# visionworkbench/visionworkbench

Hardware: AMD Instinct MI355X
Metric: disparity Mpix/s, 4096x4096 pair, 7x7 SAD, +-64-px search (higher is better)
Workload: dtype u8

## Files before the change

### visionworkbench_amd/csrc/bm_sad_u8.hip

```cpp
#include <climits>
#include <cstdlib>
#include <type_traits>

#include "vwgpu_internal.h"
#include "u8_tile.h"

#ifdef VWGPU_TILE_STAMPS
__device__ unsigned long long* g_sad_stamps = nullptr;
extern "C" int vwgpu_debug_set_sad_stamps(void* d_buf) {
  unsigned long long* p = static_cast<unsigned long long*>(d_buf);
  return hipMemcpyToSymbol(HIP_SYMBOL(g_sad_stamps), &p, sizeof p) == hipSuccess ? 0 : -3;
}
#define VWGPU_STAMP(k) do { if (g_sad_stamps && tid == 0) g_sad_stamps[(size_t)wg * 16 + (k)] = wall_clock64(); } while (0)
#else
#define VWGPU_STAMP(k) do { } while (0)
#endif

namespace {

using namespace vwgpu_u8;
typedef uint32_t u32;
typedef uint64_t u64;
typedef unsigned short u16x2 __attribute__((ext_vector_type(2)));

__device__ __forceinline__ u32 pk_sub_u16(u32 a, u32 b) {
  return __builtin_bit_cast(u32, (u16x2)(__builtin_bit_cast(u16x2, a) - __builtin_bit_cast(u16x2, b)));
}
__device__ __forceinline__ u32 pk_max_u16(u32 a, u32 b) {
  return __builtin_bit_cast(u32, __builtin_elementwise_max(__builtin_bit_cast(u16x2, a), __builtin_bit_cast(u16x2, b)));
}
__device__ __forceinline__ u32 pk_min_u16(u32 a, u32 b) {
  return __builtin_bit_cast(u32, __builtin_elementwise_min(__builtin_bit_cast(u16x2, a), __builtin_bit_cast(u16x2, b)));
}
__device__ __forceinline__ void umin3_acc(u32& k, u32 a, u32 b) {
  asm volatile("v_min3_u32 %0, %0, %1, %2" : "+v"(k) : "v"(a), "v"(b));
}

template <int W>
__device__ __forceinline__ void key_sub(u32& key, u32 a, u32 b) {
  if (W == 0)
    asm volatile("v_sub_u16_sdwa %0, %1, %2 dst_sel:WORD_1 dst_unused:UNUSED_PRESERVE src0_sel:WORD_0 src1_sel:WORD_0"
                 : "+v"(key) : "v"(a), "v"(b));
  else
    asm volatile("v_sub_u16_sdwa %0, %1, %2 dst_sel:WORD_1 dst_unused:UNUSED_PRESERVE src0_sel:WORD_1 src1_sel:WORD_1"
                 : "+v"(key) : "v"(a), "v"(b));
}

template <int KX, int KY, int TY, int WV = 0>
struct Cfg {
  static constexpr int NW = (KX + 3) / 4;
  static constexpr int EW = NW <= 2 ? 2 : 4;
  static constexpr int WAVES = WV ? WV : (NW <= 2 ? 4 : 2);
  static constexpr int THREADS = WAVES * 64;
  static constexpr int TWB = WAVES * 256;
  static constexpr int NR = TY + KY - 1;
  static constexpr int LBW = TWB / 4 + NW + 1;
  static constexpr u32 LAST_MASK = (KX % 4 == 0) ? 0xffffffffu : ((1u << (8 * (KX % 4))) - 1u);
};

__device__ __forceinline__ void divmod_small(int idx, int d, float inv, int& quo, int& rem) {
  int qq = (int)(((float)idx + 0.5f) * inv);
  int rr = idx - qq * d;
  if (rr < 0) { --qq; rr += d; }
  if (rr >= d) { ++qq; rr -= d; }
  quo = qq; rem = rr;
}

__device__ __forceinline__ bool sad_second_on_cu(unsigned block, int first_round) {
  return (int)(block >> 3) >= (first_round >> 4);
}

__host__ __device__ constexpr size_t ent_words(int nr, int ne, int ew, int gr, int ty, int pt) {
  const size_t ent = (size_t)nr * ne * ew;
  const size_t merge = gr > 1 ? (size_t)(gr - 1) * (ty / gr) * 4 * pt + (size_t)gr * pt : 0;
  const size_t ob = (size_t)gr * (pt / 64) * 768;
  return ent > merge ? (ent > ob ? ent : ob) : (merge > ob ? merge : ob);
}

template <int KX, int KY, int TY, int GR, int WV = 0, bool EM = true>
__global__ void __launch_bounds__((GR * (Cfg<KX, KY, TY, WV>::THREADS)), (GR > 1 ? 1 : (TY <= 8 && KX <= 8 ? 3 : 2)))
bm_sad_u8_kernel(const float* __restrict__ L, ptrdiff_t ls, int lw, int lh,
                 const float* __restrict__ R, ptrdiff_t rs, int rcw, int rch,
                 int sx, int sy, int ne, int32_t* __restrict__ out, ptrdiff_t os, int ow, int oh,
                 int* __restrict__ flag_set, int* __restrict__ flag_clear,
                 int gxt, int ntiles, int last_round, int first_round, int stagger_ticks) {
  typedef Cfg<KX, KY, TY, WV> C;
  constexpr bool SPLIT = GR > 1;
  constexpr int NW = C::NW, EW = C::EW, NR = C::NR;
  constexpr int NRP = EM ? (NR | 1) : NR;
  extern __shared__ __attribute__((aligned(16))) u32 lds[];
  u32* ent = lds;
  const int bpitch = ne + NW + 1;
  u32* base = lds + ent_words(NRP, ne, EW, GR, TY, C::THREADS);
  u32* item_ctr = base + (size_t)NR * bpitch;

  constexpr int PT = C::THREADS;
  constexpr int NT = GR * PT;
  const int tid = threadIdx.x;
  const int grp = SPLIT ? __builtin_amdgcn_readfirstlane(tid / PT) : 0;
  const int ltid = SPLIT ? tid % PT : tid;
  const int pair_id = __builtin_amdgcn_readfirstlane(ltid >> 6);
  const int per_xcd = gridDim.x >> 3;
  const int wg = (int)(blockIdx.x & 7) * per_xcd + (int)(blockIdx.x >> 3);
  if (wg >= ntiles) return;
  const int x0 = (wg % gxt) * C::TWB;
  const int y0 = (wg / gxt) * TY;
  const int q = x0 + 4 * ltid;
  u32 bad_acc = 0;
  if (wg == 0 && tid == 0) *flag_clear = 0;
#ifdef VWGPU_TILE_STAMPS
  if (g_sad_stamps && tid == 0) {
    unsigned hw, xcc;
    asm volatile("s_getreg_b32 %0, hwreg(HW_REG_HW_ID)" : "=s"(hw));
    asm volatile("s_getreg_b32 %0, hwreg(HW_REG_XCC_ID)" : "=s"(xcc));
    unsigned long long* rec = g_sad_stamps + (size_t)wg * 16;
    rec[0] = wall_clock64(); rec[1] = clock64(); rec[2] = ((unsigned long long)xcc << 32) | hw;
  }
#endif

  if (!SPLIT && (int)blockIdx.x < first_round && sad_second_on_cu(blockIdx.x, first_round)) {
    if (tid < 64) {
      const u64 t_start = wall_clock64();
      for (int it = 0; it < 512 && wall_clock64() - t_start < (u64)stagger_ticks; ++it) __builtin_amdgcn_s_sleep(8);
    }
    __syncthreads();
  }
  stage_u8_rows<NR>(L, ls, lw, lh, x0, y0, C::LBW, C::LBW, ent, tid, NT, bad_acc);
  stage_u8_rows<NR>(R, rs, rcw, rch, x0, y0, bpitch, bpitch, base, tid, NT, bad_acc);
  __syncthreads();
  u64 win[NR][NW];
#pragma unroll
  for (int r = 0; r < NR; ++r) {
    u32 a[NW + 1];
#pragma unroll
    for (int n = 0; n <= NW; ++n) a[n] = ent[r * C::LBW + ltid + n];
#pragma unroll
    for (int n = 0; n < NW; ++n) win[r][n] = (u64)a[n] | ((u64)a[n + 1] << 32);
  }

  VWGPU_STAMP(3);
  u32 K[TY][4];
  u32 MN[TY][2], MX[TY][2];
#pragma unroll
  for (int y = 0; y < TY; ++y) K[y][0] = K[y][1] = K[y][2] = K[y][3] = 0xffffffffu;
  u32 eq_rows = (1u << TY) - 1u;
  int eq_checks = 0;
  constexpr int NPROBE = 4;
  const u32 zero = 0;

  const bool late = !SPLIT && (int)blockIdx.x >= last_round;
  if (!SPLIT) { if (late) __builtin_amdgcn_s_setprio(2); else __builtin_amdgcn_s_setprio(3); }
  typedef std::true_type T;
  typedef std::false_type F;

  auto sweep = [&](auto max_tag) __attribute__((always_inline)) {
    constexpr bool MAXSWEEP = decltype(max_tag)::value;
    for (int dy = 0; dy < sy; ++dy) {
      __syncthreads();
      if (dy > 0 || (MAXSWEEP && sy > 1)) stage_u8_rows<NR>(R, rs, rcw, rch, x0, y0 + dy, bpitch, bpitch, base, tid, NT, bad_acc);
      for (int t = 0; t < 4; ++t) {
        const int a_last = (sx + 2 - t) >> 2;
        __syncthreads();
        if (!MAXSWEEP && !SPLIT && dy == 0 && late) {
          if (t == 2) __builtin_amdgcn_s_setprio(1);
          else if (t == 3) __builtin_amdgcn_s_setprio(0);
        }
        {
          auto build = [&](int r, int m) __attribute__((always_inline)) {
            const u32* bp = base + (size_t)r * bpitch + m;
            u32 b[NW + 1];
#pragma unroll
            for (int n = 0; n <= NW; ++n) b[n] = bp[n];
            u32 w[EW];
#pragma unroll
            for (int n = 0; n < EW; ++n) w[n] = 0;
#pragma unroll
            for (int n = 0; n < NW; ++n) w[n] = __builtin_amdgcn_alignbyte(b[n + 1], b[n], t);
            w[NW - 1] &= C::LAST_MASK;
            u32* e = ent + (EM ? (size_t)m * NRP + r : (size_t)r * ne + m) * EW;
            if (EW == 2) *reinterpret_cast<uint2*>(e) = make_uint2(w[0], w[1]);
            else *reinterpret_cast<uint4*>(e) = make_uint4(w[0], w[1], w[2 % EW], w[3 % EW]);
          };
#pragma unroll 4
          for (int r = grp; r < NR; r += NT / PT) build(r, ltid);
          const int rem = ne - PT, total = NR * rem;
          const float inv = 1.0f / (float)rem;
          for (int idx = tid; idx < total; idx += NT) {
            int r, m;
            divmod_small(idx, rem, inv, r, m);
            build(r, PT + m);
          }
          if (SPLIT && tid < PT / 64) item_ctr[tid] = 0u;
        }
        __syncthreads();

        auto step = [&](int a, auto masked_tag, auto pair_tag, auto probe_tag) __attribute__((always_inline)) {
          constexpr bool MASKED = decltype(masked_tag)::value;
          constexpr bool PAIR = decltype(pair_tag)::value;
          constexpr bool PROBE = decltype(probe_tag)::value;
          const int jbase = 4 * a + t;
          const int ibase = dy * sx + jbase;
          u32 kinA[4], kinB[4];
          u32 orA[2] = {0u, 0u};
#pragma unroll
          for (int i = 0; i < 4; ++i) {
            kinA[i] = (u32)(ibase - i) & 0xffffu;
            kinB[i] = (u32)(ibase + 4 - i) & 0xffffu;
            if (MASKED) {
              const int d = jbase - i;
              if (d < 0 || d >= sx) orA[i >> 1] |= (i & 1) ? 0xffff0000u : 0x0000ffffu;
            }
          }
          const u32* ep = ent + (size_t)(ltid + a) * (EM ? NRP * EW : EW);
          u64 accA = 0, accB = 0;
          u64 PA[NR], PB[NR];
          constexpr int PF = 4;
          u32 wa[NR][EW], wb[NR][EW];
          auto fetch = [&](int r) __attribute__((always_inline)) {
            const u32* e = ep + (EM ? (size_t)r * EW : (size_t)r * ne * EW);
            constexpr int NX = EM ? NRP * EW : EW;
            if (EW == 2) {
              const uint2 v = *reinterpret_cast<const uint2*>(e);
              wa[r][0] = v.x; wa[r][1] = v.y;
              if (PAIR) { const uint2 u = *reinterpret_cast<const uint2*>(e + NX); wb[r][0] = u.x; wb[r][1] = u.y; }
            } else {
              const uint4 v = *reinterpret_cast<const uint4*>(e);
              wa[r][0] = v.x; wa[r][1] = v.y; wa[r][2 % EW] = v.z; wa[r][3 % EW] = v.w;
              if (PAIR) { const uint4 u = *reinterpret_cast<const uint4*>(e + NX); wb[r][0] = u.x; wb[r][1] = u.y; wb[r][2 % EW] = u.z; wb[r][3 % EW] = u.w; }
            }
          };
#pragma unroll
          for (int r = 0; r < PF && r < NR; ++r) fetch(r);
#pragma unroll
          for (int r = 0; r < NR; ++r) {
            if (r + PF < NR) fetch(r + PF);
#pragma unroll
            for (int n = 0; n < NW; ++n) {
              accA = __builtin_amdgcn_qsad_pk_u16_u8(win[r][n], wa[r][n], accA);
              if (PAIR) accB = __builtin_amdgcn_qsad_pk_u16_u8(win[r][n], wb[r][n], accB);
            }
            PA[r] = accA;
            if (PAIR) PB[r] = accB;
            if (r >= KY - 1) {
              const int y = r - (KY - 1);
              const int ro = (r >= KY) ? r - KY : 0;
              const u32 nA0 = (u32)PA[r], nA1 = (u32)(PA[r] >> 32);
              const u32 oA0 = (r >= KY) ? (u32)PA[ro] : zero;
              const u32 oA1 = (r >= KY) ? (u32)(PA[ro] >> 32) : zero;
              if (MAXSWEEP) {
                const u32 sA0 = pk_sub_u16(nA0, oA0), sA1 = pk_sub_u16(nA1, oA1);
                MN[y][0] = pk_min_u16(MN[y][0], MASKED ? (sA0 | orA[0]) : sA0);
                MN[y][1] = pk_min_u16(MN[y][1], MASKED ? (sA1 | orA[1]) : sA1);
                MX[y][0] = pk_max_u16(MX[y][0], MASKED ? (sA0 & ~orA[0]) : sA0);
                MX[y][1] = pk_max_u16(MX[y][1], MASKED ? (sA1 & ~orA[1]) : sA1);
                if (PAIR) {
                  const u32 nB0 = (u32)PB[r], nB1 = (u32)(PB[r] >> 32);
                  const u32 oB0 = (r >= KY) ? (u32)PB[ro] : zero;
                  const u32 oB1 = (r >= KY) ? (u32)(PB[ro] >> 32) : zero;
                  const u32 sB0 = pk_sub_u16(nB0, oB0), sB1 = pk_sub_u16(nB1, oB1);
                  MN[y][0] = pk_min_u16(MN[y][0], sB0);
                  MN[y][1] = pk_min_u16(MN[y][1], sB1);
                  MX[y][0] = pk_max_u16(MX[y][0], sB0);
                  MX[y][1] = pk_max_u16(MX[y][1], sB1);
                }
              } else {
                key_sub<0>(kinA[0], nA0, oA0); key_sub<1>(kinA[1], nA0, oA0);
                key_sub<0>(kinA[2], nA1, oA1); key_sub<1>(kinA[3], nA1, oA1);
                if (PAIR) {
                  const u32 nB0 = (u32)PB[r], nB1 = (u32)(PB[r] >> 32);
                  const u32 oB0 = (r >= KY) ? (u32)PB[ro] : zero;
                  const u32 oB1 = (r >= KY) ? (u32)(PB[ro] >> 32) : zero;
                  key_sub<0>(kinB[0], nB0, oB0); key_sub<1>(kinB[1], nB0, oB0);
                  key_sub<0>(kinB[2], nB1, oB1); key_sub<1>(kinB[3], nB1, oB1);
                  if (PROBE) {
                    u32 x[4];
#pragma unroll
                    for (int i = 0; i < 4; ++i) {
                      asm volatile("v_xor_b32 %0, %1, %2" : "=v"(x[i]) : "v"(kinA[i]), "v"(kinB[i]));
                      x[i] = (q + i < ow) ? x[i] : 0xffffffffu;
                    }
                    const u32 m01 = x[0] < x[1] ? x[0] : x[1], m23 = x[2] < x[3] ? x[2] : x[3];
                    if ((m01 < m23 ? m01 : m23) >> 16) eq_rows &= ~(1u << y);
                  }
                  umin3_acc(K[y][0], kinA[0], kinB[0]);
                  umin3_acc(K[y][1], kinA[1], kinB[1]);
                  umin3_acc(K[y][2], kinA[2], kinB[2]);
                  umin3_acc(K[y][3], kinA[3], kinB[3]);
                } else {
                  const u32 kA0 = (MASKED && (orA[0] & 0x0000ffffu)) ? 0xffffffffu : kinA[0];
                  const u32 kA1 = (MASKED && (orA[0] & 0xffff0000u)) ? 0xffffffffu : kinA[1];
                  const u32 kA2 = (MASKED && (orA[1] & 0x0000ffffu)) ? 0xffffffffu : kinA[2];
                  const u32 kA3 = (MASKED && (orA[1] & 0xffff0000u)) ? 0xffffffffu : kinA[3];
                  umin3_acc(K[y][0], kA0, kA0);
                  umin3_acc(K[y][1], kA1, kA1);
                  umin3_acc(K[y][2], kA2, kA2);
                  umin3_acc(K[y][3], kA3, kA3);
                }
              }
            }
          }
        };

        int a_lo = (t >= 3) ? 0 : 1;
        int a_hi = (sx - 1 - t >= 0) ? ((sx - 1 - t) >> 2) + 1 : 0;
        if (a_hi > a_last + 1) a_hi = a_last + 1;
        if (a_lo > a_hi) a_lo = a_hi;
        const int n1 = a_lo;
        const int npair = (a_hi - n1) > 0 ? (a_hi - n1) >> 1 : 0;
        int nprobe = 0;
        if (!MAXSWEEP && dy == 0 && t == 0) nprobe = npair < NPROBE - eq_checks ? npair : NPROBE - eq_checks;
        const int a4 = n1 + 2 * npair;
        const int n4 = a_last - a4 + 1 > 0 ? a_last - a4 + 1 : 0;
        const int nitems = n1 + npair + n4;
        int seq = 0;
        auto next_item = [&]() __attribute__((always_inline)) -> int {
          if (MAXSWEEP) return grp == 0 ? seq++ : 0x7fffffff;
          if (!SPLIT) return seq++;
          int lane, v = 0;
          asm volatile("v_mbcnt_lo_u32_b32 %0, -1, 0\n\tv_mbcnt_hi_u32_b32 %0, -1, %0" : "=v"(lane));
          if (lane == 0) v = (int)atomicAdd(&item_ctr[pair_id], 1u);
          return __builtin_amdgcn_readfirstlane(v);
        };
        int i = next_item();
        for (; i < n1; i = next_item()) step(i, T{}, F{}, F{});
        for (; i < n1 + nprobe; i = next_item()) step(n1 + 2 * (i - n1), F{}, T{}, T{});
        for (; i < n1 + npair; i = next_item()) step(n1 + 2 * (i - n1), F{}, T{}, F{});
        for (; i < nitems; i = next_item()) step(a4 + (i - n1 - npair), T{}, F{}, F{});
        eq_checks += nprobe;
        if (!MAXSWEEP && dy == 0) VWGPU_STAMP(4 + t);
      }
    }
  };
  sweep(F{});
  if (!SPLIT) __builtin_amdgcn_s_setprio(3);

  if (bad_acc != 0u) atomicOr(flag_set, 1);
  constexpr int RG = TY / GR;
  static_assert(TY % GR == 0, "rows per group");
  auto row_mine = [&](int y) __attribute__((always_inline)) -> bool { return !SPLIT || (y / RG == grp); };
  if (SPLIT) {
    u32* xk = ent;
    u32* xe = ent + (size_t)(GR - 1) * RG * 4 * PT;
    u32 eq_all = eq_rows;
#pragma unroll
    for (int d = 0; d < GR; ++d) {
      __syncthreads();
      if (grp != d) {
        const int slot = grp < d ? grp : grp - 1;
#pragma unroll
        for (int y = 0; y < RG; ++y)
#pragma unroll
          for (int s2 = 0; s2 < 4; ++s2) xk[((slot * RG + y) * 4 + s2) * PT + ltid] = K[d * RG + y][s2];
      }
      if (d == 0) xe[grp * PT + ltid] = eq_rows;
      __syncthreads();
      if (grp == d) {
#pragma unroll
        for (int slot = 0; slot < GR - 1; ++slot)
#pragma unroll
          for (int y = 0; y < RG; ++y)
#pragma unroll
            for (int s2 = 0; s2 < 4; ++s2) {
              const u32 o = xk[((slot * RG + y) * 4 + s2) * PT + ltid];
              K[d * RG + y][s2] = o < K[d * RG + y][s2] ? o : K[d * RG + y][s2];
            }
      }
      if (d == 0) {
#pragma unroll
        for (int g2 = 0; g2 < GR; ++g2) eq_all &= xe[g2 * PT + ltid];
      }
    }
    eq_rows = eq_all;
  }
  u32 cand = eq_checks < NPROBE ? (1u << TY) - 1u : eq_rows;
#pragma unroll
  for (int y = 0; y < TY; ++y)
    if (y0 + y >= oh || q >= ow || !row_mine(y)) cand &= ~(1u << y);
  const int any = __syncthreads_or(cand != 0u);

  {
    const int wv = ltid >> 6, lane = ltid & 63;
    u32* ob = ent + (size_t)(grp * (PT / 64) + wv) * 768;
    const int xw = x0 + 256 * wv;
    int nd = (ow - xw) * 3;
    nd = nd < 0 ? 0 : (nd > 768 ? 768 : nd);
    const u32 sx_magic = sx > 1 ? (u32)(0xffffffffu / (u32)sx) + 1u : 0u;
    struct __attribute__((packed, aligned(4))) U4 { u32 x, y, z, w; };
#pragma unroll
    for (int y = 0; y < TY; ++y) {
      const int oy = y0 + y;
      if (oy >= oh || !row_mine(y)) continue;
      u32 v[12];
#pragma unroll
      for (int s = 0; s < 4; ++s) {
        const u32 di = K[y][s] & 0xffffu;
        u32 dx, dy;
        if (sy == 1) { dx = di; dy = 0; }
        else { dy = sx == 1 ? di : __umulhi(di, sx_magic); dx = di - dy * (u32)sx; }
        v[3 * s] = dx;
        v[3 * s + 1] = dy;
        v[3 * s + 2] = 0x7fffffffu;
      }
      uint4* ow4 = reinterpret_cast<uint4*>(ob + lane * 12);
      ow4[0] = make_uint4(v[0], v[1], v[2], v[3]);
      ow4[1] = make_uint4(v[4], v[5], v[6], v[7]);
      ow4[2] = make_uint4(v[8], v[9], v[10], v[11]);
      int32_t* orow = out + ((ptrdiff_t)oy * os + xw) * 3;
#pragma unroll
      for (int k = 0; k < 3; ++k) {
        const int idx = k * 256 + lane * 4;
        const uint4 t = *reinterpret_cast<const uint4*>(ob + idx);
        if (idx + 3 < nd) {
          U4 u; u.x = t.x; u.y = t.y; u.z = t.z; u.w = t.w;
          *reinterpret_cast<U4*>(orow + idx) = u;
        } else {
          if (idx < nd) orow[idx] = (int32_t)t.x;
          if (idx + 1 < nd) orow[idx + 1] = (int32_t)t.y;
          if (idx + 2 < nd) orow[idx + 2] = (int32_t)t.z;
        }
      }
    }
  }

#ifdef VWGPU_TILE_STAMPS
  if (g_sad_stamps && tid == 0) { g_sad_stamps[(size_t)wg * 16 + 8] = wall_clock64(); g_sad_stamps[(size_t)wg * 16 + 9] = clock64(); }
#endif
  if (__builtin_expect(!any, 1)) return;
#pragma unroll
  for (int y = 0; y < TY; ++y) {
    MN[y][0] = MN[y][1] = 0xffffffffu;
    MX[y][0] = MX[y][1] = 0u;
  }
  sweep(T{});
  if (grp == 0) {
#pragma unroll
    for (int y = 0; y < TY; ++y) {
      const u32 same0 = MN[y][0] ^ MX[y][0], same1 = MN[y][1] ^ MX[y][1];
      const bool inv[4] = {(same0 & 0xffffu) == 0, (same0 >> 16) == 0, (same1 & 0xffffu) == 0, (same1 >> 16) == 0};
#pragma unroll
      for (int s = 0; s < 4; ++s)
        if (inv[s] && y0 + y < oh && q + s < ow)
          out[((ptrdiff_t)(y0 + y) * os + q + s) * 3 + 2] = 0;
    }
  }
}

typedef void (*KernelFn)(const float*, ptrdiff_t, int, int, const float*, ptrdiff_t, int, int, int, int, int,
                         int32_t*, ptrdiff_t, int, int, int*, int*, int, int, int, int, int);
struct Launch {
  int kx, ky, ty;
  int threads, twb, nr, ew, nw;
  int split_groups;
  KernelFn fn;
  KernelFn split_fn;
  KernelFn fn_rm, split_fn_rm;
};

template <bool ON, int KX, int KY, int TY, int GR, int WV, bool EM>
constexpr KernelFn kernel_if() {
  if constexpr (ON) return bm_sad_u8_kernel<KX, KY, TY, GR, WV, EM>;
  else return nullptr;
}

template <int KX, int KY, int TY, bool WITH_SPLIT = false, int WV = 0>
constexpr Launch make_launch() {
  typedef Cfg<KX, KY, TY, WV> C;
  return Launch{KX, KY, TY, C::THREADS, C::TWB, C::NR, C::EW, C::NW, WV ? 4 : 2,
                kernel_if<WV == 0, KX, KY, TY, 1, WV, true>(),
                kernel_if<WITH_SPLIT, KX, KY, TY, (WV ? 4 : 2), WV, true>(),
                kernel_if<WV == 0, KX, KY, TY, 1, WV, false>(),
                kernel_if<WITH_SPLIT, KX, KY, TY, (WV ? 4 : 2), WV, false>()};
}

const Launch kLaunch[] = {
    make_launch<3, 3, 16>(), make_launch<5, 5, 16>(), make_launch<7, 7, 16, true>(), make_launch<7, 7, 8, true>(), make_launch<7, 7, 16, true, 2>(),
    make_launch<7, 5, 16>(), make_launch<9, 9, 12>(), make_launch<11, 11, 8>(),
};

const Launch* find_launch(int kx, int ky) {
  for (const Launch& l : kLaunch)
    if (l.kx == kx && l.ky == ky) return &l;
  return nullptr;
}

const Launch* pick_launch(int kx, int ky, int ow, int oh, int num_cu, int groups, bool* split) {
  const Launch* best = nullptr;
  double best_cost = 0.0;
  *split = false;
  if (groups == 3) {
    bool has = false;
    for (const Launch& l : kLaunch) has |= l.kx == kx && l.ky == ky && l.split_fn && !l.fn;
    if (!has) groups = 0;
  }
  for (const Launch& l : kLaunch) {
    if (l.kx != kx || l.ky != ky) continue;
    const long long wgs = (long long)((ow + l.twb - 1) / l.twb) * ((oh + l.ty - 1) / l.ty);
    const double n = (double)((wgs + num_cu - 1) / num_cu);
    const int resident = (l.ty <= 8 && l.kx <= 8) ? 3 : 2;
    const bool narrow = l.twb * 2 <= 4 * 256 && l.split_fn && !l.fn;
    const double wfrac = narrow ? 0.5 : 1.0;
    for (int sp = 0; sp < 2; ++sp) {
      if (sp && !l.split_fn) continue;
      if (!sp && !l.fn) continue;
      if (groups == 3 && !narrow) continue;
      if (groups && groups != 3 && (narrow || (l.split_fn && (groups == 2) != (sp == 1)))) continue;
      const double steps = (sp ? l.nr * 0.55 * n : (n < 2.0 ? l.nr * 0.74 : l.nr * 0.5 * n)) * wfrac;
      const double rounds = sp ? n : (double)(((long long)n + resident - 1) / resident);
      const double cost = steps + (narrow ? 5.7 : 4.5) * rounds;
      if (!best || cost < best_cost) { best = &l; best_cost = cost; *split = sp != 0; }
    }
  }
  return best;
}

constexpr size_t kMaxLds = 80 * 1024;

constexpr int kStaggerTicks = 1400;

int entries_per_row(const Launch& l, int sx) { return l.twb / 4 + ((sx + 2) >> 2) + 1; }

size_t lds_bytes(const Launch& l, int sx, int groups, bool em) {
  const int ne = entries_per_row(l, sx);
  const size_t ent = ent_words(em ? (l.nr | 1) : l.nr, ne, l.ew, groups, l.ty, l.threads);
  const size_t left = (size_t)l.nr * (l.twb / 4 + l.nw + 1);
  const size_t base = (size_t)l.nr * (ne + l.nw + 1);
  return ((ent > left ? ent : left) + base) * sizeof(u32);
}

bool supported(const vwgpu_bm_args& a) {
  if (a.cost_type != VWGPU_ABSOLUTE_DIFFERENCE) return false;
  const Launch* l = find_launch(a.kx, a.ky);
  if (!l) return false;
  if ((long long)a.sx * a.sy > 65535) return false;
  return lds_bytes(*l, a.sx, l->split_fn ? l->split_groups : 1, false) <= kMaxLds;
}

int launch(vwgpu_ctx* ctx, const vwgpu_bm_args& a, int** d_flag) {
  const int kx = a.kx, sx = a.sx, sy = a.sy, ow = a.ow(), oh = a.oh();
  bool split = false;
  const int plan_cu = ctx->sad_round_slots > 0 ? (ctx->sad_round_slots + 1) / 2 : ctx->num_cu;
  const Launch* l = pick_launch(kx, a.ky, ow, oh, plan_cu, ctx->sad_groups, &split);
  if (!l) return vwgpu_fail(ctx, VWGPU_ERR_NOIMPL, "no packed-u8 kernel for %dx%d", kx, a.ky);
  const int rcw = a.lw + sx - 1, rch = a.lh + sy - 1;
  const int gx = (ow + l->twb - 1) / l->twb, gy = (oh + l->ty - 1) / l->ty;
  const int ne = entries_per_row(*l, sx);
  const int groups = split ? l->split_groups : 1;
  const size_t ctr_bytes = split ? 64 : 0;
  const bool em = ctx->sad_layout == 0 && lds_bytes(*l, sx, groups, true) + ctr_bytes <= kMaxLds;
  const size_t shmem = lds_bytes(*l, sx, groups, em) + ctr_bytes;
  ctx->sad_last_launch = l->ty | (l->twb / 256) << 8 | groups << 12 | (em ? 1 : 0) << 16;
  const KernelFn main_fn = em ? (split ? l->split_fn : l->fn) : (split ? l->split_fn_rm : l->fn_rm);
  const unsigned grid1 = (unsigned)((gx * gy + 7) / 8 * 8);
  const int resident = (l->ty <= 8 && l->kx <= 8) ? 3 : 2;
  const int slots = ctx->sad_round_slots > 0 ? ctx->sad_round_slots : ctx->num_cu * resident;
  const bool rounds = !split && (int)grid1 >= 2 * slots;
  const int last_round = rounds ? (int)grid1 - slots : INT_MAX;
  const int first_round = (rounds && resident == 2) ? slots : 0;
  vwgpu_flag_pair f;
  int rc = vwgpu_packed_prologue(ctx, reinterpret_cast<const void*>(main_fn), shmem, d_flag, &f);
  if (rc) return rc;
  {
    vwgpu_prof_scope ps(ctx, "bm_sad_u8");
    hipLaunchKernelGGL(main_fn, dim3(grid1), dim3(split ? l->split_groups * l->threads : l->threads), shmem, ctx->stream,
                       a.left, a.ls, a.lw, a.lh, a.right, a.rs, rcw, rch, sx, sy, ne, a.out, a.os, ow, oh,
                       f.set, f.clear, gx, gx * gy, last_round, first_round, kStaggerTicks);
  }
  VWGPU_HIP(ctx, hipGetLastError());
  return VWGPU_OK;
}

}

vwgpu_bm_matcher vwgpu_bm_sad_u8 = {VWGPU_PATH_SAD_U8, 7, "packed-u8", supported, launch};
```

### visionworkbench_amd/csrc/u8_tile.h

```cpp
#pragma once
#include <hip/hip_runtime.h>
#include <cstdint>

namespace vwgpu_u8 {

typedef uint32_t u32;

__device__ __forceinline__ u32 pack4_check(float4 v, u32& acc) {
  u32 p = 0;
  p = __builtin_amdgcn_cvt_pk_u8_f32(v.x, 0, p);
  p = __builtin_amdgcn_cvt_pk_u8_f32(v.y, 1, p);
  p = __builtin_amdgcn_cvt_pk_u8_f32(v.z, 2, p);
  p = __builtin_amdgcn_cvt_pk_u8_f32(v.w, 3, p);
  acc |= __builtin_bit_cast(u32, v.x - (float)(p & 0xffu));
  acc |= __builtin_bit_cast(u32, v.y - (float)((p >> 8) & 0xffu));
  acc |= __builtin_bit_cast(u32, v.z - (float)((p >> 16) & 0xffu));
  acc |= __builtin_bit_cast(u32, v.w - (float)(p >> 24));
  return p;
}

template <int NROWS>
__device__ __forceinline__ void patch_right_edge(const float* __restrict__ img, ptrdiff_t stride, int w, int h,
                                                 int x0, int y0, int ndw, int dst_pitch_dw,
                                                 u32* __restrict__ dst, int tid, int nthreads, u32& acc) {
  const int ge = (w - x0) >> 2;
  if (ge >= 0 && ge < ndw && ((w - x0) & 3) != 0) {
    for (int r = tid; r < NROWS; r += nthreads) {
      const int y = y0 + r;
      u32 p = 0;
      if (y < h) {
        const float* row = img + (ptrdiff_t)y * stride;
        const int x = x0 + 4 * ge;
        const float4 v = make_float4(row[x], x + 1 < w ? row[x + 1] : 0.0f, x + 2 < w ? row[x + 2] : 0.0f, 0.0f);
        p = pack4_check(v, acc);
      }
      dst[r * dst_pitch_dw + ge] = p;
    }
  }
}

template <int NROWS>
struct U8MainLoads { float4 v[NROWS]; };

struct __attribute__((packed, aligned(4))) F4U { float x, y, z, w; };
__device__ __forceinline__ float4 load_f4(const float* p) {
  const F4U u = *reinterpret_cast<const F4U*>(p);
  return make_float4(u.x, u.y, u.z, u.w);
}

template <int NROWS>
__device__ __forceinline__ void stage_u8_main_issue(const float* __restrict__ img, ptrdiff_t stride, int w, int h, int x0, int y0, int ndw,
                                                    int tid, U8MainLoads<NROWS>& ld) {
  if (tid < ndw) {
    const int x = x0 + 4 * tid;
    const int off = (x + 3 < w) ? x : 0;
    const int hv = w >= 4 ? h : 0;
#pragma unroll
    for (int r = 0; r < NROWS; ++r) {
      const float* rowp = (y0 + r < hv) ? img + (ptrdiff_t)(y0 + r) * stride : img;
      ld.v[r] = load_f4(rowp + off);
    }
  }
}
template <int NROWS>
__device__ __forceinline__ void stage_u8_main_finish(int w, int h, int x0, int y0, int ndw, int dst_pitch_dw, u32* __restrict__ dst, int tid,
                                                     const U8MainLoads<NROWS>& ld, u32& acc) {
  if (tid < ndw) {
    const int g = tid, x = x0 + 4 * g;
    const bool colin = x + 3 < w;
#pragma unroll
    for (int r = 0; r < NROWS; ++r) {
      u32 a = 0;
      const u32 p = pack4_check(ld.v[r], a);
      const bool inb = colin && (y0 + r < h);
      if (inb) acc |= a;
      if (colin || x >= w) dst[r * dst_pitch_dw + g] = inb ? p : 0u;
    }
  }
}

template <int NROWS>
__device__ __forceinline__ void stage_u8_rest(const float* __restrict__ img, ptrdiff_t stride, int w, int h,
                                              int x0, int y0, int ndw, int dst_pitch_dw,
                                              u32* __restrict__ dst, int tid, int nthreads, u32& acc) {
  const int rem = ndw - nthreads;
  if (rem > 0) {
    const int total = NROWS * rem;
    const float inv = 1.0f / (float)rem;
    for (int i0 = 0; i0 < total; i0 += 4 * nthreads) {
      float4 v[4]; int di[4]; bool inb[4];
#pragma unroll
      for (int k = 0; k < 4; ++k) {
        const int idx = i0 + k * nthreads + tid;
        int r = (int)(((float)(idx < total ? idx : 0) + 0.5f) * inv);
        int c = (idx < total ? idx : 0) - r * rem;
        if (c < 0) { --r; c += rem; }
        if (c >= rem) { ++r; c -= rem; }
        const int g = nthreads + c, x = x0 + 4 * g;
        inb[k] = (idx < total) && (x + 3 < w) && (y0 + r < h);
        di[k] = (idx < total && (x + 3 < w || x >= w)) ? r * dst_pitch_dw + g : -1;
        const float* src = inb[k] ? img + (ptrdiff_t)(y0 + r) * stride + x : img;
        v[k] = load_f4(src);
      }
#pragma unroll
      for (int k = 0; k < 4; ++k) {
        u32 a = 0;
        const u32 p = pack4_check(v[k], a);
        if (inb[k]) acc |= a;
        if (di[k] >= 0) dst[di[k]] = inb[k] ? p : 0u;
      }
    }
  }
  patch_right_edge<NROWS>(img, stride, w, h, x0, y0, ndw, dst_pitch_dw, dst, tid, nthreads, acc);
}

template <int NROWS>
__device__ __forceinline__ void stage_u8_rows(const float* __restrict__ img, ptrdiff_t stride, int w, int h,
                                              int x0, int y0, int ndw, int dst_pitch_dw,
                                              u32* __restrict__ dst, int tid, int nthreads, u32& acc) {
  U8MainLoads<NROWS> ld;
  stage_u8_main_issue<NROWS>(img, stride, w, h, x0, y0, ndw, tid, ld);
  stage_u8_main_finish<NROWS>(w, h, x0, y0, ndw, dst_pitch_dw, dst, tid, ld, acc);
  stage_u8_rest<NROWS>(img, stride, w, h, x0, y0, ndw, dst_pitch_dw, dst, tid, nthreads, acc);
}

}
```

Measured before the change: 52670.

## Pair masked tail steps, use SDWA equality probes, and strength-reduce margin divmod

Result: no change. 53010 (median of 6 runs) (+0.7%).

```diff
diff --git a/visionworkbench_amd/csrc/bm_sad_u8.hip b/visionworkbench_amd/csrc/bm_sad_u8.hip
--- a/visionworkbench_amd/csrc/bm_sad_u8.hip
+++ b/visionworkbench_amd/csrc/bm_sad_u8.hip
@@ -153,11 +153,17 @@
   typedef std::true_type T;
   typedef std::false_type F;
 
+  const float margin_inv = 1.0f / (float)(ne - PT);
+  int margin_dr, margin_dm;
+  divmod_small(NT, ne - PT, margin_inv, margin_dr, margin_dm);
+  margin_dr = __builtin_amdgcn_readfirstlane(margin_dr);
+  margin_dm = __builtin_amdgcn_readfirstlane(margin_dm);
+
   auto sweep = [&](auto max_tag) __attribute__((always_inline)) {
     constexpr bool MAXSWEEP = decltype(max_tag)::value;
     for (int dy = 0; dy < sy; ++dy) {
       __syncthreads();
-      if (dy > 0 || (MAXSWEEP && sy > 1)) stage_u8_rows<NR>(R, rs, rcw, rch, x0, y0 + dy, bpitch, bpitch, base, tid, NT, bad_acc);
+      if (dy > 0 || (MAXSWEEP && sy > 1)) stage_u8_rows<NR, false>(R, rs, rcw, rch, x0, y0 + dy, bpitch, bpitch, base, tid, NT, bad_acc);
       for (int t = 0; t < 4; ++t) {
         const int a_last = (sx + 2 - t) >> 2;
         __syncthreads();
@@ -183,17 +189,21 @@
           };
 #pragma unroll 4
           for (int r = grp; r < NR; r += NT / PT) build(r, ltid);
-          const int rem = ne - PT, total = NR * rem;
-          const float inv = 1.0f / (float)rem;
-          for (int idx = tid; idx < total; idx += NT) {
-            int r, m;
-            divmod_small(idx, rem, inv, r, m);
+          const int rem = ne - PT;
+          int r, m;
+          divmod_small(tid, rem, margin_inv, r, m);
+          while (r < NR) {
             build(r, PT + m);
+            r += margin_dr; m += margin_dm;
+            if (m >= rem) { m -= rem; ++r; }
           }
           if (SPLIT && tid < PT / 64) item_ctr[tid] = 0u;
         }
         __syncthreads();
 
+        u64 eq_lanes[TY];
+#pragma unroll
+        for (int y = 0; y < TY; ++y) eq_lanes[y] = ~0ull;
         auto step = [&](int a, auto masked_tag, auto pair_tag, auto probe_tag) __attribute__((always_inline)) {
           constexpr bool MASKED = decltype(masked_tag)::value;
           constexpr bool PAIR = decltype(pair_tag)::value;
@@ -201,14 +211,17 @@
           const int jbase = 4 * a + t;
           const int ibase = dy * sx + jbase;
           u32 kinA[4], kinB[4];
-          u32 orA[2] = {0u, 0u};
+          u32 orA[2] = {0u, 0u}, orB[2] = {0u, 0u};
+          u32 offA[4], offB[4];
 #pragma unroll
           for (int i = 0; i < 4; ++i) {
             kinA[i] = (u32)(ibase - i) & 0xffffu;
             kinB[i] = (u32)(ibase + 4 - i) & 0xffffu;
+            offA[i] = offB[i] = 0u;
             if (MASKED) {
               const int d = jbase - i;
-              if (d < 0 || d >= sx) orA[i >> 1] |= (i & 1) ? 0xffff0000u : 0x0000ffffu;
+              if (d < 0 || d >= sx) { orA[i >> 1] |= (i & 1) ? 0xffff0000u : 0x0000ffffu; offA[i] = 0xffff0000u; }
+              if (PAIR && (d + 4 < 0 || d + 4 >= sx)) { orB[i >> 1] |= (i & 1) ? 0xffff0000u : 0x0000ffffu; offB[i] = 0xffff0000u; }
             }
           }
           const u32* ep = ent + (size_t)(ltid + a) * (EM ? NRP * EW : EW);
@@ -258,10 +271,10 @@
                   const u32 oB0 = (r >= KY) ? (u32)PB[ro] : zero;
                   const u32 oB1 = (r >= KY) ? (u32)(PB[ro] >> 32) : zero;
                   const u32 sB0 = pk_sub_u16(nB0, oB0), sB1 = pk_sub_u16(nB1, oB1);
-                  MN[y][0] = pk_min_u16(MN[y][0], sB0);
-                  MN[y][1] = pk_min_u16(MN[y][1], sB1);
-                  MX[y][0] = pk_max_u16(MX[y][0], sB0);
-                  MX[y][1] = pk_max_u16(MX[y][1], sB1);
+                  MN[y][0] = pk_min_u16(MN[y][0], MASKED ? (sB0 | orB[0]) : sB0);
+                  MN[y][1] = pk_min_u16(MN[y][1], MASKED ? (sB1 | orB[1]) : sB1);
+                  MX[y][0] = pk_max_u16(MX[y][0], MASKED ? (sB0 & ~orB[0]) : sB0);
+                  MX[y][1] = pk_max_u16(MX[y][1], MASKED ? (sB1 & ~orB[1]) : sB1);
                 }
               } else {
                 key_sub<0>(kinA[0], nA0, oA0); key_sub<1>(kinA[1], nA0, oA0);
@@ -273,14 +286,24 @@
                   key_sub<0>(kinB[0], nB0, oB0); key_sub<1>(kinB[1], nB0, oB0);
                   key_sub<0>(kinB[2], nB1, oB1); key_sub<1>(kinB[3], nB1, oB1);
                   if (PROBE) {
-                    u32 x[4];
+                    u64 c[4];
+#pragma unroll
+                    for (int i = 0; i < 4; ++i)
+                      asm volatile("v_cmp_eq_u16_sdwa %0, %1, %2 src0_sel:WORD_1 src1_sel:WORD_1" : "=s"(c[i]) : "v"(kinA[i]), "v"(kinB[i]));
+                    if (SPLIT) {
+                      u32 bit;
+                      asm("v_cndmask_b32_e64 %0, %1, 0, %2" : "=v"(bit) : "v"(1u << y), "s"((c[0] | c[1]) | (c[2] | c[3])));
+                      eq_rows &= ~bit;
+                    } else {
+                      eq_lanes[y] &= (c[0] | c[1]) | (c[2] | c[3]);
+                    }
+                  }
+                  if (MASKED) {
 #pragma unroll
                     for (int i = 0; i < 4; ++i) {
-                      asm volatile("v_xor_b32 %0, %1, %2" : "=v"(x[i]) : "v"(kinA[i]), "v"(kinB[i]));
-                      x[i] = (q + i < ow) ? x[i] : 0xffffffffu;
+                      asm volatile("v_or_b32 %0, %1, %0" : "+v"(kinA[i]) : "s"(offA[i]));
+                      asm volatile("v_or_b32 %0, %1, %0" : "+v"(kinB[i]) : "s"(offB[i]));
                     }
-                    const u32 m01 = x[0] < x[1] ? x[0] : x[1], m23 = x[2] < x[3] ? x[2] : x[3];
-                    if ((m01 < m23 ? m01 : m23) >> 16) eq_rows &= ~(1u << y);
                   }
                   umin3_acc(K[y][0], kinA[0], kinB[0]);
                   umin3_acc(K[y][1], kinA[1], kinB[1]);
@@ -311,7 +334,8 @@
         if (!MAXSWEEP && dy == 0 && t == 0) nprobe = npair < NPROBE - eq_checks ? npair : NPROBE - eq_checks;
         const int a4 = n1 + 2 * npair;
         const int n4 = a_last - a4 + 1 > 0 ? a_last - a4 + 1 : 0;
-        const int nitems = n1 + npair + n4;
+        const int ntail = (n4 + 1) >> 1;
+        const int nitems = n1 + npair + ntail;
         int seq = 0;
         auto next_item = [&]() __attribute__((always_inline)) -> int {
           if (MAXSWEEP) return grp == 0 ? seq++ : 0x7fffffff;
@@ -324,8 +348,19 @@
         int i = next_item();
         for (; i < n1; i = next_item()) step(i, T{}, F{}, F{});
         for (; i < n1 + nprobe; i = next_item()) step(n1 + 2 * (i - n1), F{}, T{}, T{});
+        if (!MAXSWEEP && !SPLIT && nprobe > 0) {
+          u32 dropped = 0;
+#pragma unroll
+          for (int y = 0; y < TY; ++y) {
+            u32 bit;
+            asm("v_cndmask_b32_e64 %0, %1, 0, %2" : "=v"(bit) : "v"(1u << y), "s"(eq_lanes[y]));
+            dropped |= bit;
+          }
+          eq_rows &= ~dropped;
+        }
         for (; i < n1 + npair; i = next_item()) step(n1 + 2 * (i - n1), F{}, T{}, F{});
-        for (; i < nitems; i = next_item()) step(a4 + (i - n1 - npair), T{}, F{}, F{});
+        for (; i < n1 + npair + (n4 >> 1); i = next_item()) step(a4 + 2 * (i - n1 - npair), T{}, T{}, F{});
+        for (; i < nitems; i = next_item()) step(a4 + (n4 & ~1), T{}, F{}, F{});
         eq_checks += nprobe;
         if (!MAXSWEEP && dy == 0) VWGPU_STAMP(4 + t);
       }
diff --git a/visionworkbench_amd/csrc/u8_tile.h b/visionworkbench_amd/csrc/u8_tile.h
--- a/visionworkbench_amd/csrc/u8_tile.h
+++ b/visionworkbench_amd/csrc/u8_tile.h
@@ -12,10 +12,11 @@
   p = __builtin_amdgcn_cvt_pk_u8_f32(v.y, 1, p);
   p = __builtin_amdgcn_cvt_pk_u8_f32(v.z, 2, p);
   p = __builtin_amdgcn_cvt_pk_u8_f32(v.w, 3, p);
-  acc |= __builtin_bit_cast(u32, v.x - (float)(p & 0xffu));
-  acc |= __builtin_bit_cast(u32, v.y - (float)((p >> 8) & 0xffu));
-  acc |= __builtin_bit_cast(u32, v.z - (float)((p >> 16) & 0xffu));
-  acc |= __builtin_bit_cast(u32, v.w - (float)(p >> 24));
+  const u32 dx = __builtin_bit_cast(u32, v.x) ^ __builtin_bit_cast(u32, (float)(p & 0xffu));
+  const u32 dy = __builtin_bit_cast(u32, v.y) ^ __builtin_bit_cast(u32, (float)((p >> 8) & 0xffu));
+  const u32 dz = __builtin_bit_cast(u32, v.z) ^ __builtin_bit_cast(u32, (float)((p >> 16) & 0xffu));
+  const u32 dw = __builtin_bit_cast(u32, v.w) ^ __builtin_bit_cast(u32, (float)(p >> 24));
+  acc = (acc | dx | dy) | (dz | dw);
   return p;
 }
 
@@ -62,19 +63,29 @@
     }
   }
 }
-template <int NROWS>
+template <int NROWS, bool INTERIOR = true>
 __device__ __forceinline__ void stage_u8_main_finish(int w, int h, int x0, int y0, int ndw, int dst_pitch_dw, u32* __restrict__ dst, int tid,
                                                      const U8MainLoads<NROWS>& ld, u32& acc) {
   if (tid < ndw) {
     const int g = tid, x = x0 + 4 * g;
     const bool colin = x + 3 < w;
+    if (INTERIOR && y0 + NROWS <= h) {
+      if (colin) {
 #pragma unroll
-    for (int r = 0; r < NROWS; ++r) {
-      u32 a = 0;
-      const u32 p = pack4_check(ld.v[r], a);
-      const bool inb = colin && (y0 + r < h);
-      if (inb) acc |= a;
-      if (colin || x >= w) dst[r * dst_pitch_dw + g] = inb ? p : 0u;
+        for (int r = 0; r < NROWS; ++r) dst[r * dst_pitch_dw + g] = pack4_check(ld.v[r], acc);
+      } else if (x >= w) {
+#pragma unroll
+        for (int r = 0; r < NROWS; ++r) dst[r * dst_pitch_dw + g] = 0u;
+      }
+    } else {
+#pragma unroll
+      for (int r = 0; r < NROWS; ++r) {
+        u32 a = 0;
+        const u32 p = pack4_check(ld.v[r], a);
+        const bool inb = colin && (y0 + r < h);
+        if (inb) acc |= a;
+        if (colin || x >= w) dst[r * dst_pitch_dw + g] = inb ? p : 0u;
+      }
     }
   }
 }
@@ -114,13 +125,13 @@
   patch_right_edge<NROWS>(img, stride, w, h, x0, y0, ndw, dst_pitch_dw, dst, tid, nthreads, acc);
 }
 
-template <int NROWS>
+template <int NROWS, bool INTERIOR = true>
 __device__ __forceinline__ void stage_u8_rows(const float* __restrict__ img, ptrdiff_t stride, int w, int h,
                                               int x0, int y0, int ndw, int dst_pitch_dw,
                                               u32* __restrict__ dst, int tid, int nthreads, u32& acc) {
   U8MainLoads<NROWS> ld;
   stage_u8_main_issue<NROWS>(img, stride, w, h, x0, y0, ndw, tid, ld);
-  stage_u8_main_finish<NROWS>(w, h, x0, y0, ndw, dst_pitch_dw, dst, tid, ld, acc);
+  stage_u8_main_finish<NROWS, INTERIOR>(w, h, x0, y0, ndw, dst_pitch_dw, dst, tid, ld, acc);
   stage_u8_rest<NROWS>(img, stride, w, h, x0, y0, ndw, dst_pitch_dw, dst, tid, nthreads, acc);
 }
 
```
